# ctu-vras/monoforce

Hardware: AMD Instinct MI355X
Metric: rollout-steps/sec (batch x horizon) on 256x256 terrain (higher is better)
Workload: dtype f32; 1 GPU; c3: B=1024/GPU x T=500 x N=4 contact points, 256x256 grid (res 0.05 m), one shared terrain+friction map (the same on every rank), integrator=odeint-euler (reference default), forward+backward; BASE...; rollouts_per_gpu=1024, rollouts_total=1024, horizon=500, contact_points=4, parallelism=rollout-sharded x1

## Files before the change

monoforce_amd/csrc/rollout_fwd_cp_kernel.h:

```cpp
#pragma once
#include "rollout_cp_common.h"
#include "rollout_fwd_kernel.h"
#include <type_traits>

namespace mf {

template <typename S, int INTEG, bool FORCES, bool ZMU, bool REC, bool LOSS = false>
__global__ void __launch_bounds__(256) __attribute__((amdgpu_waves_per_eu(1, 2))) rollout_fwd_cp_kernel(const RolloutArgs<S> a) {
  using namespace cp;
  using M = Mth<S, std::is_same<S, float>::value>;
  using Msk = typename MaskOf<S>::type;
  constexpr unsigned kS = (unsigned)sizeof(S);
  const int tid = blockIdx.x * blockDim.x + threadIdx.x;
  const int b = (tid >> 4) + a.b0;
  if (b >= a.B) return;
  if (a.loss_poison != nullptr && tid == 0) a.loss_poison[0] = (S)__builtin_nanf("");
  const int p = (tid >> 2) & 3;
  const int q = tid & 3;
  const int cc = q < 3 ? q : 2;
  const S one = S(1.0), zero = S(0.0);
  const int HW = a.H * a.W, last = HW - 1;
  const bool has_mu = a.mu != nullptr;
  const unsigned moff = a.map_shared ? 0u : (unsigned)b * (unsigned)HW;
  const S* zmap = a.z;
  const S* mumap = has_mu ? a.mu : a.z;

  const bool act = p < a.N;
  const int pi = act ? p : 0;
  const S P0 = a.points[pi * 3 + 0], P1 = a.points[pi * 3 + 1], P2 = a.points[pi * 3 + 2];
  const int part = act ? a.part[pi] : -1;
  const S tv_v = part < 0 ? zero : one;
  const S tv_w = part < 0 ? zero : ((part & 1) ? a.half_ly : -a.half_ly);
  const S I0 = a.Iinv[cc * 3 + 0], I1 = a.Iinv[cc * 3 + 1], I2 = a.Iinv[cc * 3 + 2];
  const S grav_c = cc == 2 ? a.mg * a.inv_mass : zero;
  const int cell_off = ((q & 1) ? a.H : 0) + ((q & 2) ? 1 : 0);
  const S wa_s = (q & 2) ? one : -one, wa_o = (q & 2) ? zero : one;
  const S wb_s = (q & 1) ? one : -one, wb_o = (q & 1) ? zero : one;
  const S n_mul = q < 2 ? -a.inv_res : zero, n_add = q < 2 ? zero : one;

  S x, xd, w, R0, R1, R2;
  if (a.default_state) {
    const S v0 = a.controls[(size_t)b * a.ctrl_sb + 0], w0 = a.controls[(size_t)b * a.ctrl_sb + 1];
    x = zero; xd = cc == 0 ? v0 : zero; w = cc == 2 ? w0 : zero;
    R0 = cc == 0 ? one : zero; R1 = cc == 1 ? one : zero; R2 = cc == 2 ? one : zero;
    if (p == 0) {
      S* oxd = const_cast<S*>(a.xd0); S* oR = const_cast<S*>(a.R0); S* ow = const_cast<S*>(a.w0);
      a.x0[b * 3 + cc] = x; oxd[b * 3 + cc] = xd; ow[b * 3 + cc] = w;
      oR[b * 9 + cc * 3 + 0] = R0; oR[b * 9 + cc * 3 + 1] = R1; oR[b * 9 + cc * 3 + 2] = R2;
    }
  } else {
    x = a.x0[b * 3 + cc]; xd = a.xd0[b * 3 + cc]; w = a.w0[b * 3 + cc];
    R0 = a.R0[b * 9 + cc * 3 + 0]; R1 = a.R0[b * 9 + cc * 3 + 1]; R2 = a.R0[b * 9 + cc * 3 + 2];
  }

  auto footprint = [&](S pc, int* idx, S* wq, S* ou = nullptr) {
    const S lim = S(262144.0);
    const S u = M::cell_coord(pc, a.d_max, a.res, a.inv_res);
    const int ui = (int)M::clamp(u, -lim, lim);
    const S fr = u - (S)ui;
    const int base = dppi<kB1>(ui) + __mul24(a.H, dppi<kB0>(ui));
    *idx = min(max(base + cell_off, 0), last);
    const S wa = mf_fma(wa_s, dpp<kB0>(fr), wa_o), wb = mf_fma(wb_s, dpp<kB1>(fr), wb_o);
    *wq = wa * wb;
    if (ou) *ou = u;
  };

  if (!a.skip_snap) {
    const S pc = (P0 * R0 + P1 * R1 + P2 * R2) + x;
    int idx; S wq;
    footprint(pc, &idx, &wq);
    const S zq = dot4(wq, ld32(zmap, moff + (unsigned)idx));
    const S acc = sum_points(act ? zq : zero);
    const S xz = acc / (S)a.N;
    x = cc == 2 ? xz : x;
    if (p == 0 && q == 2) a.x0[b * 3 + 2] = xz;
  }

  const unsigned row_stride = (a.layout == MF_LAYOUT_TIME_MAJOR) ? (unsigned)a.B : 1u;
  const unsigned row0 = (a.layout == MF_LAYOUT_TIME_MAJOR) ? (unsigned)b : (unsigned)b * (unsigned)a.T;
  S* v3base = p == 0 ? a.Xs : p == 1 ? a.Xds : p == 2 ? a.Om : (a.Xraw ? a.Xraw : a.Xs);
  const S sink_l = (p == 3 && a.Xraw) ? zero : a.sink;
  const Msk m_xd = p == 1 ? ~(Msk)0 : (Msk)0, m_w = p == 2 ? ~(Msk)0 : (Msk)0;
  char* p3 = reinterpret_cast<char*>(v3base) + (size_t)(row0 * 3u + (unsigned)cc) * kS;
  const Rsrc rCtrl = make_rsrc(a.controls);
  unsigned o9 = (row0 * 9u + (unsigned)cc * 3u) * kS;
  const unsigned frow = (unsigned)a.fstride * 3u;
  unsigned ofs = (row0 * frow + (unsigned)p * 3u + (unsigned)cc) * kS, off = ofs;
  const unsigned d3 = row_stride * 3u * kS, d9 = row_stride * 9u * kS, df = row_stride * frow * kS;
  const char* pRs = reinterpret_cast<const char*>(a.Rs);
  const char* pFs = reinterpret_cast<const char*>(a.Fs);
  const char* pFf = reinterpret_cast<const char*>(a.Ff);

  S oFs = zero, oFf = zero;

  auto emit_row = [&](S ex, S exd, S ew, S e0, S e1, S e2, unsigned adv) {
    const S vx = mf_fma(e2, sink_l, ex);
    const S v3 = bfi(m_w, ew, bfi(m_xd, exd, vx));
    __builtin_nontemporal_store(v3, reinterpret_cast<S*>(p3));
    bstore3(pRs, o9, 0u, e0, e1, e2);
    if (FORCES) { bstore1(pFs, ofs, 0u, oFs); bstore1(pFf, off, 0u, oFf); }
    if (adv) { p3 += d3; o9 += d9; ofs += df; off += df; }
  };

  const int n_steps = (INTEG == MF_INTEG_ODEINT_EULER) ? a.T - 1 : a.T;
  unsigned v_ctrl = (unsigned)b * (unsigned)a.ctrl_sb * kS;
  S cv, cw;
  bload2(rCtrl, v_ctrl, 0u, &cv, &cw);
  S h_ode = (INTEG == MF_INTEG_ODEINT_EULER && a.T > 1) ? a.ts[1] - a.ts[0] : zero;
  struct Geo { S r, pc, wq, zc, mc, e, u, il, coln2; int idx; };
  auto geometry = [&](S gx, S g0, S g1, S g2) {
    Geo g;
    g.r = cp_body_r(P0, P1, P2, g0, g1, g2);
    g.pc = g.r + gx;
    footprint(g.pc, &g.idx, &g.wq, &g.u);
    const int idx = g.idx;
    if constexpr (ZMU) {
      const Pk2<S> zm = *reinterpret_cast<const Pk2<S>*>(reinterpret_cast<const char*>(a.zmu) + (size_t)((unsigned)idx * 2u * kS));
      g.zc = zm.a; g.mc = zm.b;
    } else {
      g.zc = ld32(zmap, moff + (unsigned)idx);
      g.mc = ld32(mumap, moff + (unsigned)idx);
    }
    g.coln2 = dot3(g0, g0);
    g.il = M::inv_len(g.coln2);
    g.e = g0 * g.il;
    return g;
  };
  char* const pRec0 = reinterpret_cast<char*>(a.rec);
  unsigned rec_off = (unsigned)tid * kRecBytesPerLane<S>;
  const unsigned rec_step = (unsigned)a.B * 16u * kRecBytesPerLane<S>;
  typedef S f4v __attribute__((ext_vector_type(4)));
  auto rec_store = [&](const f4v& rq, unsigned adv) {
#if defined(MF_REC_NOSTORE)
    asm volatile("" :: "v"(rq));
#elif defined(MF_REC_PLAIN)
    *reinterpret_cast<f4v*>(pRec0 + (size_t)rec_off) = rq;
#else
    __builtin_nontemporal_store(rq, reinterpret_cast<f4v*>(pRec0 + (size_t)rec_off));
#endif
    if (adv) rec_off += rec_step;
  };
  auto contact = [&](const Geo& g, S vxd, S vw, S tv, S* xdd, S* wd, S* oFr, S* oFf, f4v* rq) {
    const S vp = cp_vel(vxd, vw, g.r);
    const S zq = dot4(g.wq, g.zc);
    const S mub = dot4(g.wq, has_mu ? g.mc : one);
    const S dz = g.zc - dpp<kB0>(g.zc);
    const S u = mf_fma(dpp<kN12>(dz), n_mul, n_add);
    const S inl = M::inv_len(dot3(u, u));
    const S nrm = u * inl;
    const S dh = dpp<kB2>(g.pc) - zq;
    S cj = M::sigmoid_m10(dh);
    cj = act ? cj : zero;
    const S csum = sum_points(cj);
    const S inv_csum = M::div(one, csum);
    const S vn = dot3(vp, nrm);
    const S A = cp_normal_force(a.k, dh, a.damp, vn);
    const S Fr = M::clamp(cp_spring(A, nrm, cj, inv_csum), -a.mg, a.mg);
    const S Nn = M::sqrt(dot3(Fr, Fr));
    const S s = mub * cp_cmd(tv, g.e, vp);
    const S sn = dot3(s, nrm);
    const S Ff = M::clamp(Nn * cp_tangent(s, sn, nrm), -a.mg, a.mg);
    const S f = Fr + Ff;
    const S tau = unrot(cross_pre(g.r, f));
    const S Fsum = sum_points(f), Tsum = sum_points(tau);
    const S wraw = cp_wraw(I0, I1, I2, Tsum);
    *wd = M::clamp(wraw, -a.omega_max, a.omega_max);
    *xdd = Fsum * a.inv_mass - grav_c;
    *oFr = Fr; *oFf = Ff;
    if constexpr (REC) *rq = f4v{g.u, cj, wraw, A};
  };

  S l_acc = zero;
  int l_j = 0;
  const int l_last = LOSS ? a.loss_T2 - 1 : 0;
  const unsigned l_lane = LOSS ? ((unsigned)b * (unsigned)a.loss_T2 * 3u + (unsigned)cc) : 0u;
  struct Stamp { S g, w; };
  auto loss_peek = [&](int row) {
    Stamp st = {zero, zero};
    if constexpr (LOSS) {
      st.g = ld32(a.loss_gt, l_lane + (unsigned)(min(l_j, l_last) * 3));
      st.w = a.loss_row_w[row];
    }
    return st;
  };
  auto loss_row = [&](S ex, S e2, const Stamp& st) {
    if constexpr (LOSS) {
      const S term = cp_loss_term(mf_fma(e2, a.sink, ex), st.g, st.w);
      l_acc += st.w != zero ? term : zero;
      l_j += st.w != zero ? 1 : 0;
    }
  };

  if constexpr (INTEG == MF_INTEG_ODEINT_EULER) {
    S t_cur = a.T > 1 ? a.ts[1] : zero;
    const unsigned ctrl_step = (unsigned)a.ctrl_st * kS, v_ctrl_last = v_ctrl + (unsigned)(a.T - 1) * ctrl_step;
    unsigned v_ts = kS;
    asm("" : "+v"(v_ts));
    const unsigned v_ts_last = (unsigned)max(a.T - 1, 0) * kS;
    auto ode_step = [&](int n, const Geo& g, Geo& g_next, S cv_n, S cw_n, S h, S& cv_next, S& cw_next, S& h_next) {
      v_ctrl = min(v_ctrl + ctrl_step, v_ctrl_last);
      bload2(rCtrl, v_ctrl, 0u, &cv_next, &cw_next);
      v_ts = min(v_ts + kS, v_ts_last);
      const S t_next = *reinterpret_cast<const S*>(reinterpret_cast<const char*>(a.ts) + (size_t)v_ts);
      const Stamp stamp = loss_peek(n + 1);
      const S tv = cp_track(tv_v, tv_w, cv_n, cw_n);
      const S d0 = h * cross_pre(w, R0), d1 = h * cross_pre(w, R1), d2 = h * cross_pre(w, R2);
      const S xn = mf_fma(h, xd, x);
      const S Rn0 = R0 + unrot(d0), Rn1 = R1 + unrot(d1), Rn2 = R2 + unrot(d2);
      g_next = geometry(xn, Rn0, Rn1, Rn2);
      emit_row(x, xd, w, R0, R1, R2, 1u);
      x = xn; R0 = Rn0; R1 = Rn1; R2 = Rn2;
      S xdd, wd, Fr, Ff;
      f4v rq;
      contact(g, xd, w, tv, &xdd, &wd, &Fr, &Ff, &rq);
      if constexpr (REC) rec_store(rq, 1u);
      xd = mf_fma(h, xdd, xd);
      w = mf_fma(h, wd, w);
      oFs = mf_fma(h, Fr, oFs);
      oFf = mf_fma(h, Ff, oFf);
      h_next = t_next - t_cur;
      t_cur = t_next;
      loss_row(x, R2, stamp);
    };
    Geo gA, gB;
    S cvA = cv, cwA = cw, hA = h_ode, cvB = zero, cwB = zero, hB = zero;
    if (n_steps > 0) gA = geometry(x, R0, R1, R2);
    loss_row(x, R2, loss_peek(0));
    __builtin_amdgcn_s_waitcnt(0);
    int n = 0;
    for (; n + 1 < n_steps; n += 2) {
      ode_step(n, gA, gB, cvA, cwA, hA, cvB, cwB, hB);
      ode_step(n + 1, gB, gA, cvB, cwB, hB, cvA, cwA, hA);
    }
    if (n < n_steps) ode_step(n, gA, gB, cvA, cwA, hA, cvB, cwB, hB);
  } else {
    __builtin_amdgcn_s_waitcnt(0);
    for (int n = 0; n < n_steps; ++n) {
      const int nn = min(n + 1, a.T - 1);
      S cv_next, cw_next;
      bload2(rCtrl, v_ctrl, __builtin_amdgcn_readfirstlane((unsigned)(nn * a.ctrl_st) * kS), &cv_next, &cw_next);
      const S tv = cp_track(tv_v, tv_w, cv, cw);
      S xdd, wd, Fr, Ff;
      const Geo g = geometry(x, R0, R1, R2);
      emit_row(x, xd, w, R0, R1, R2, n > 0 ? 1u : 0u);
      f4v rq;
      contact(g, xd, w, tv, &xdd, &wd, &Fr, &Ff, &rq);
      if constexpr (REC) rec_store(rq, 1u);
      const S h = a.dt;
      xd = mf_fma(xdd, h, xd);
      x = mf_fma(xd, h, x);
      w = mf_fma(wd, h, w);
      const S th2 = dot3(w, w);
      const S il = M::inv_len(th2);
      const S kc = w * il;
      const S k1 = dpp<kRot1>(kc), k2 = dpp<kRot2>(kc);
      S sn_, oc;
      M::sincos_small(M::len_of(th2, il) * h, &sn_, &oc);
      const S kk = M::kReciprocalNorm ? th2 * (il * il) : dot3(kc, kc);
      const S ock = oc * kc;
      const S m0 = one + oc * (kc * kc - kk);
      const S m1 = mf_fma(ock, k1, -(sn_ * k2));
      const S m2 = mf_fma(ock, k2, sn_ * k1);
      const S n0 = R0 * dpp<kB0>(m0) + R1 * dpp<kB1>(m2) + R2 * dpp<kB2>(m1);
      const S n1 = R0 * dpp<kB0>(m1) + R1 * dpp<kB1>(m0) + R2 * dpp<kB2>(m2);
      const S n2 = R0 * dpp<kB0>(m2) + R1 * dpp<kB1>(m1) + R2 * dpp<kB2>(m0);
      R0 = n0; R1 = n1; R2 = n2;
      oFs = Fr; oFf = Ff;
      cv = cv_next; cw = cw_next;
    }
  }
  if (n_steps > 0 || INTEG == MF_INTEG_ODEINT_EULER) emit_row(x, xd, w, R0, R1, R2, 1u);
  if constexpr (LOSS) {
    static_assert(!LOSS || INTEG == MF_INTEG_ODEINT_EULER, "the fused loss rides on the default integrator's kernels");
    __shared__ S l_sh[80];
    const int lane = threadIdx.x;
    if (lane < 16) l_sh[lane] = zero;
    if (p == 0 && q < 3) l_sh[(lane >> 4) * 4 + q] = l_acc;
    __syncthreads();
    unsigned last = 0u;
    if (lane == 0) {
      S tot = zero;
#pragma unroll
      for (int r = 0; r < 4; ++r) tot += (l_sh[r * 4 + 0] + l_sh[r * 4 + 1]) + l_sh[r * 4 + 2];
      __builtin_nontemporal_store(tot, a.loss_partial + blockIdx.x);
      __threadfence();
      last = atomicAdd(a.loss_ticket, 1u) == gridDim.x - 1 ? 1u : 0u;
    }
    last = __builtin_amdgcn_readfirstlane(last);
    if (last) {
      __threadfence();
      const int n_act = min(64, (a.B - (int)blockIdx.x * 4) * 16);
      S tot = zero;
      for (unsigned k2 = (unsigned)lane; k2 < gridDim.x; k2 += (unsigned)n_act) tot += __builtin_nontemporal_load(a.loss_partial + k2);
      l_sh[16 + lane] = tot;
      __syncthreads();
      if (lane == 0) {
        S sum = zero;
        for (int k2 = 0; k2 < n_act; ++k2) sum += l_sh[16 + k2];
        a.loss_out[0] = sum * a.loss_inv_count;
        *a.loss_ticket = 0u;
      }
    }
  }
}

int launch_rollout_fwd_cp_f32(const RolloutArgs<float>& a, const FwdRoute& r, int integ, hipStream_t st);
int launch_rollout_fwd_cp_f64(const RolloutArgs<double>& a, const FwdRoute& r, int integ, hipStream_t st);
template <typename S>
int launch_rollout_fwd_cp_t(const RolloutArgs<S>& a, const FwdRoute& r, int integ, hipStream_t st) {
  const int block = r.block;
  const unsigned grid = (unsigned)(((long long)a.B * 16 + block - 1) / block);
  const bool forces = r.forces, zmu = r.zmu;
  const bool rec = r.record;
  if (r.loss == kLossInLaunch) {
    constexpr int I = MF_INTEG_ODEINT_EULER;
    if (rec) { if (zmu) MF_KLAUNCH((rollout_fwd_cp_kernel<S, I, false, true, true, true>), dim3(grid), dim3(block), 0, st, a);
               else MF_KLAUNCH((rollout_fwd_cp_kernel<S, I, false, false, true, true>), dim3(grid), dim3(block), 0, st, a); }
    else     { if (zmu) MF_KLAUNCH((rollout_fwd_cp_kernel<S, I, false, true, false, true>), dim3(grid), dim3(block), 0, st, a);
               else MF_KLAUNCH((rollout_fwd_cp_kernel<S, I, false, false, false, true>), dim3(grid), dim3(block), 0, st, a); }
    hipError_t e = hipGetLastError();
    MF_REQUIRE(e == hipSuccess, MF_ERR_LAUNCH, std::string("rollout_fwd (component-parallel, fused loss) launch: ") + hipGetErrorString(e));
    return MF_OK;
  }
#define MF_CP(INTEG_, FORCES_, ZMU_) do { if (rec) MF_KLAUNCH((rollout_fwd_cp_kernel<S, INTEG_, FORCES_, ZMU_, true>), dim3(grid), dim3(block), 0, st, a); \
                                          else MF_KLAUNCH((rollout_fwd_cp_kernel<S, INTEG_, FORCES_, ZMU_, false>), dim3(grid), dim3(block), 0, st, a); } while (0)
#define MF_CP_F(INTEG_)                                          \
  do {                                                           \
    if (forces) { if (zmu) MF_CP(INTEG_, true, true); else MF_CP(INTEG_, true, false); }    \
    else        { if (zmu) MF_CP(INTEG_, false, true); else MF_CP(INTEG_, false, false); }  \
  } while (0)
  if (integ == MF_INTEG_DYNAMICS) MF_CP_F(MF_INTEG_DYNAMICS); else MF_CP_F(MF_INTEG_ODEINT_EULER);
#undef MF_CP_F
#undef MF_CP
  hipError_t e = hipGetLastError();
  MF_REQUIRE(e == hipSuccess, MF_ERR_LAUNCH, std::string("rollout_fwd (component-parallel) launch: ") + hipGetErrorString(e));
  return MF_OK;
}


}
```

monoforce_amd/csrc/rollout_fwd_kernel.h:

```cpp
#pragma once
#include <cstdlib>
#include "rollout_common.h"
#include "rollout_route.h"

namespace mf {

template <typename S>
struct RolloutArgs {
  int B, T, N, H, W, n_tracks, layout, map_shared, skip_snap, fstride, default_state, ctrl_sb, ctrl_st, b0;
  S mass, inv_mass, mg, k, damp, omega_max, res, inv_res, d_max, dt, half_ly, sink;
  S Iinv[9];
  const S* z;
  const S* mu;
  const S* controls;
  const S* ts;
  const S* points;
  const int* part;
  S* x0;
  const S* xd0;
  const S* R0;
  const S* w0;
  S* Xs;
  S* Xds;
  S* Rs;
  S* Om;
  S* Fs;
  S* Ff;
  S* Xraw;
  const S* joint_angles;
  S joint_xyz[12];
  S* cost_rows;
  int pose_stride;
  S* path_cost;
  const S* zmu;
  S* rec;
  int loss_T2;
  const S* loss_gt;
  const S* loss_row_w;
  S* loss_partial;
  unsigned* loss_ticket;
  S* loss_out;
  S loss_inv_count;
  S* loss_poison;
};

template <typename S, bool FAST>
struct Mth {
  static __device__ __forceinline__ S div(S a, S b) { return a / b; }
  static __device__ __forceinline__ S cell_coord(S q, S d_max, S res, S) { return (q + d_max) / res; }
  static __device__ __forceinline__ S sqrt(S v) { return mf_sqrt(v); }
  static __device__ __forceinline__ S sigmoid_m10(S dh) { return (S)1 / ((S)1 + mf_exp((S)10 * dh)); }
  static __device__ __forceinline__ S inv_len(S len2) { return (S)1 / mf_max(mf_sqrt(len2), (S)1e-6); }
  static __device__ __forceinline__ S len_of(S len2, S) { return mf_sqrt(len2); }
  static constexpr bool kReciprocalNorm = false;
  static __device__ __forceinline__ void sincos_small(S v, S* s, S* omc) { S c; mf_sincos(v, s, &c); *omc = (S)1 - c; }
  static __device__ __forceinline__ S clamp(S v, S lo, S hi) { return mf_clamp(v, lo, hi); }
  static __device__ __forceinline__ void sincos(S v, S* sn, S* cs) { mf_sincos(v, sn, cs); }
};
template <>
struct Mth<float, true> {
  static __device__ __forceinline__ float div(float a, float b) { return a * __builtin_amdgcn_rcpf(b); }
  static __device__ __forceinline__ float cell_coord(float q, float d_max, float res, float inv_res) {
    const float a = q + d_max;
    const float u = a * inv_res;
    return fmaf(fmaf(-u, res, a), inv_res, u);
  }
  static __device__ __forceinline__ float sqrt(float v) { return __builtin_amdgcn_sqrtf(v); }
  static __device__ __forceinline__ float sigmoid_m10(float dh) {
    return __builtin_amdgcn_rcpf(1.0f + __builtin_amdgcn_exp2f(14.426950408889634f * dh));
  }
  static __device__ __forceinline__ float inv_len(float len2) { return __builtin_amdgcn_rsqf(fmaxf(len2, 1e-12f)); }
  static __device__ __forceinline__ float len_of(float len2, float il) { return len2 * il; }
  static constexpr bool kReciprocalNorm = true;
  static __device__ __forceinline__ float clamp(float v, float lo, float hi) { return __builtin_amdgcn_fmed3f(v, lo, hi); }
  static __device__ __forceinline__ void sincos(float v, float* sn, float* cs) { *sn = __sinf(v); *cs = __cosf(v); }
  static __device__ __forceinline__ void sincos_small(float v, float* s, float* omc) {
    const float v2 = v * v;
    const float ts = v * (1.0f + v2 * (-1.0f / 6 + v2 * (1.0f / 120 - v2 * (1.0f / 5040))));
    const float tc = v2 * (0.5f + v2 * (-1.0f / 24 + v2 * (1.0f / 720 - v2 * (1.0f / 40320))));
    const float rev = __builtin_amdgcn_fractf(v * 0.15915494309189535f);
    const bool small = fabsf(v) < 0.25f;
    *s = small ? ts : __builtin_amdgcn_sinf(rev);
    *omc = small ? tc : 1.0f - __builtin_amdgcn_cosf(rev);
  }
};

template <typename S, bool FAST>
__device__ __forceinline__ Cell<S> locate_m(S qx, S qy, S d_max, S res, S inv_res, int H, int last) {
  const S lim = (S)262144.0;
  S ux = Mth<S, FAST>::cell_coord(qx, d_max, res, inv_res);
  S uy = Mth<S, FAST>::cell_coord(qy, d_max, res, inv_res);
  int ix = (int)Mth<S, FAST>::clamp(ux, -lim, lim);
  int iy = (int)Mth<S, FAST>::clamp(uy, -lim, lim);
  Cell<S> c;
  c.fx = ux - (S)ix;
  c.fy = uy - (S)iy;
  int base = iy + __mul24(H, ix);
  c.ic = min(max(base, 0), last);
  c.i_f = min(max(base + H, 0), last);
  c.il = min(max(base + 1, 0), last);
  c.ifl = min(max(base + 1 + H, 0), last);
  return c;
}

template <typename S>
__device__ __forceinline__ S ld32(const S* base, unsigned elem) {
  return *reinterpret_cast<const S*>(reinterpret_cast<const char*>(base) + (size_t)(elem * (unsigned)sizeof(S)));
}

template <typename S>
struct CellPair { S a, b; };
template <typename S>
__device__ __forceinline__ void gather4(const S* map, unsigned moff, const Cell<S>& c, int last, S (&v)[4]) {
  const int p1 = min(c.ic, last - 1), p2 = min(c.i_f, last - 1);
  const CellPair<S> q1 = *reinterpret_cast<const CellPair<S>*>(reinterpret_cast<const char*>(map) + (size_t)((moff + (unsigned)p1) * (unsigned)sizeof(S)));
  const CellPair<S> q2 = *reinterpret_cast<const CellPair<S>*>(reinterpret_cast<const char*>(map) + (size_t)((moff + (unsigned)p2) * (unsigned)sizeof(S)));
  v[0] = c.ic != p1 ? q1.b : q1.a;
  v[2] = c.il != p1 ? q1.b : q1.a;
  v[1] = c.i_f != p2 ? q2.b : q2.a;
  v[3] = c.ifl != p2 ? q2.b : q2.a;
}

template <typename S>
struct CellQuad { S za, ma, zb, mb; };
template <typename S>
__device__ __forceinline__ void gather4x2(const S* zmu, const Cell<S>& c, int last, S (&z)[4], S (&m)[4]) {
  const int p1 = min(c.ic, last - 1), p2 = min(c.i_f, last - 1);
  const CellQuad<S> q1 = *reinterpret_cast<const CellQuad<S>*>(reinterpret_cast<const char*>(zmu) + (size_t)((unsigned)p1 * (unsigned)(2 * sizeof(S))));
  const CellQuad<S> q2 = *reinterpret_cast<const CellQuad<S>*>(reinterpret_cast<const char*>(zmu) + (size_t)((unsigned)p2 * (unsigned)(2 * sizeof(S))));
  const bool ec = c.ic != p1, el = c.il != p1, ef = c.i_f != p2, efl = c.ifl != p2;
  z[0] = ec ? q1.zb : q1.za;   m[0] = ec ? q1.mb : q1.ma;
  z[2] = el ? q1.zb : q1.za;   m[2] = el ? q1.mb : q1.ma;
  z[1] = ef ? q2.zb : q2.za;   m[1] = ef ? q2.mb : q2.ma;
  z[3] = efl ? q2.zb : q2.za;  m[3] = efl ? q2.mb : q2.ma;
}

template <typename S, int G, int PPL, bool FAST = false>
__device__ __forceinline__ void articulate_body(GroupSum<G, S>& gs, const S* ja, const S* joint_xyz, S mp, const S (&P0)[PPL][3],
                                                const int (&part)[PPL], const bool (&act)[PPL], S (&P)[PPL][3], S (&Iv)[9]) {
  const S one = (S)1, zero = (S)0;
  S sj[4], cj4[4];
#pragma unroll
  for (int q = 0; q < 4; ++q) Mth<S, FAST>::sincos(ja[q], &sj[q], &cj4[q]);
  S I6[6] = {zero, zero, zero, zero, zero, zero};
#pragma unroll
  for (int j = 0; j < PPL; ++j) {
    const int q = max(part[j], 0);
    const S sn = sj[q], cs = cj4[q];
    const S jx = joint_xyz[q * 3 + 0], jz = joint_xyz[q * 3 + 2];
    const S dx = P0[j][0] - jx, dz = P0[j][2] - jz;
    const S rx = (dx * cs + dz * sn) + jx, rz = (-(dx * sn) + dz * cs) + jz;
    P[j][0] = part[j] >= 0 ? rx : P0[j][0];
    P[j][1] = P0[j][1];
    P[j][2] = part[j] >= 0 ? rz : P0[j][2];
    const S px = P[j][0], py = P[j][1], pzz = P[j][2];
    const S wgt = act[j] ? mp : zero;
    I6[0] += wgt * (py * py + pzz * pzz); I6[1] += wgt * (px * px + pzz * pzz); I6[2] += wgt * (px * px + py * py);
    I6[3] -= wgt * px * py; I6[4] -= wgt * px * pzz; I6[5] -= wgt * py * pzz;
  }
  gs.sum_n(I6);
  const S a00 = I6[0], a11 = I6[1], a22 = I6[2], a01 = I6[3], a02 = I6[4], a12 = I6[5];
  const S c00 = a11 * a22 - a12 * a12, c01 = a02 * a12 - a01 * a22, c02 = a01 * a12 - a02 * a11;
  const S c11 = a00 * a22 - a02 * a02, c12 = a01 * a02 - a00 * a12, c22 = a00 * a11 - a01 * a01;
  const S idet = Mth<S, FAST>::div(one, a00 * c00 + a01 * c01 + a02 * c02);
  Iv[0] = c00 * idet; Iv[1] = c01 * idet; Iv[2] = c02 * idet;
  Iv[3] = c01 * idet; Iv[4] = c11 * idet; Iv[5] = c12 * idet;
  Iv[6] = c02 * idet; Iv[7] = c12 * idet; Iv[8] = c22 * idet;
}

template <typename S, int G, int PPL, int INTEG, bool FAST, bool JOINTS = false, bool FORCES = true, int COST = 0, bool SPLIT = false, bool ZMU = false, bool REC = false>
__global__ void __launch_bounds__(G > 256 ? G : 256) rollout_fwd_kernel(const RolloutArgs<S> a) {
  using M = Mth<S, FAST>;
  const int tid = blockIdx.x * blockDim.x + threadIdx.x;
  const int b = tid / G + a.b0;
  const int gl = tid % G;
  if (b >= a.B) return;
  const S one = (S)1, zero = (S)0;
  const int HW = a.H * a.W, last = HW - 1;
  const bool has_mu = a.mu != nullptr;
  __shared__ S gs_lds[G > 64 ? 2 * (G / 64) * kGroupSumMaxValues : 1];
  GroupSum<G, S> gs;
  gs.lds = gs_lds;
  const unsigned moff = a.map_shared ? 0u : (unsigned)b * (unsigned)HW;
  const S* zmap = a.z;
  const S* mumap = has_mu ? a.mu : a.z;

  S P[PPL][3];
  S P0[PPL][3];
  S Iv[9];
  int part[PPL];
  bool act[PPL];
#pragma unroll
  for (int j = 0; j < PPL; ++j) {
    int i = gl * PPL + j;
    act[j] = i < a.N;
    int ii = act[j] ? i : 0;
    P[j][0] = a.points[ii * 3 + 0];
    P[j][1] = a.points[ii * 3 + 1];
    P[j][2] = a.points[ii * 3 + 2];
    part[j] = act[j] ? a.part[ii] : -1;
#pragma unroll
    for (int c = 0; c < 3; ++c) P0[j][c] = P[j][c];
  }
#pragma unroll
  for (int c = 0; c < 9; ++c) Iv[c] = a.Iinv[c];

  S x[3], xd[3], R[9], w[3];
  if (a.default_state) {
    const S v0 = a.controls[(size_t)b * a.ctrl_sb + 0], w0 = a.controls[(size_t)b * a.ctrl_sb + 1];
#pragma unroll
    for (int c = 0; c < 3; ++c) { x[c] = zero; xd[c] = c == 0 ? v0 : zero; w[c] = c == 2 ? w0 : zero; }
#pragma unroll
    for (int c = 0; c < 9; ++c) R[c] = (c % 4 == 0) ? one : zero;
    if (gl == 0) {
      S* oxd = const_cast<S*>(a.xd0); S* oR = const_cast<S*>(a.R0); S* ow = const_cast<S*>(a.w0);
#pragma unroll
      for (int c = 0; c < 3; ++c) { a.x0[b * 3 + c] = x[c]; oxd[b * 3 + c] = xd[c]; ow[b * 3 + c] = w[c]; }
#pragma unroll
      for (int c = 0; c < 9; ++c) oR[b * 9 + c] = R[c];
    }
  } else {
#pragma unroll
    for (int c = 0; c < 3; ++c) {
      x[c] = a.x0[b * 3 + c];
      xd[c] = a.xd0[b * 3 + c];
      w[c] = a.w0[b * 3 + c];
    }
#pragma unroll
    for (int c = 0; c < 9; ++c) R[c] = a.R0[b * 9 + c];
  }

  if (!a.skip_snap) {
    S acc = zero;
#pragma unroll
    for (int j = 0; j < PPL; ++j) {
      S px = P[j][0] * R[0] + P[j][1] * R[1] + P[j][2] * R[2] + x[0];
      S py = P[j][0] * R[3] + P[j][1] * R[4] + P[j][2] * R[5] + x[1];
      Cell<S> c = locate_m<S, FAST>(px, py, a.d_max, a.res, a.inv_res, a.H, last);
      S z4[4];
      gather4(zmap, moff, c, last, z4);
      S v = blend(c, z4[0], z4[1], z4[2], z4[3]);
      acc += act[j] ? v : zero;
    }
    acc = gs.sum(acc);
    x[2] = acc / (S)a.N;
    if (gl == 0) a.x0[b * 3 + 2] = x[2];
  }

  const size_t row_stride = (a.layout == MF_LAYOUT_TIME_MAJOR) ? (size_t)a.B : 1;
  const size_t row0 = (a.layout == MF_LAYOUT_TIME_MAJOR) ? (size_t)b : (size_t)b * a.T;
  S* pXs = a.Xs + row0 * 3;
  S* pXds = a.Xds + row0 * 3;
  S* pOm = a.Om + row0 * 3;
  S* pRs = a.Rs + row0 * 9;
  S* pXraw = (a.Xraw ? a.Xraw : a.Xs) + row0 * 3;
  const size_t frow = (size_t)a.fstride * 3;
  S* pFs = a.Fs + row0 * frow + (size_t)gl * PPL * 3;
  S* pFf = a.Ff + row0 * frow + (size_t)gl * PPL * 3;

  S oFs[PPL][3], oFf[PPL][3];
#pragma unroll
  for (int j = 0; j < PPL; ++j)
#pragma unroll
    for (int c = 0; c < 3; ++c) oFs[j][c] = oFf[j][c] = zero;

  S* pC = COST ? a.cost_rows + row0 * 4 : nullptr;
  const int role = gl & 3;
  const bool role_b0 = (role & 1) != 0, role_b1 = (role & 2) != 0;
  const S sink_l = (role == 0 && a.Xraw) ? zero : a.sink;
  S* pV3 = role == 0 ? pXraw : role == 1 ? pXs : role == 2 ? pXds : pOm;
  S* pRrow = pRs + 3 * min(role, 2);
  int pose_wait = 0;
  S pc_n = zero, pc_mean = zero, pc_m2 = zero;
  auto store_pose = [&]() {
    pXs[0] = x[0] + R[2] * a.sink; pXs[1] = x[1] + R[5] * a.sink; pXs[2] = x[2] + R[8] * a.sink;
#pragma unroll
    for (int c = 0; c < 9; ++c) pRs[c] = R[c];
  };
  const S inv_N = one / (S)a.N, inv_Nm1 = one / (S)max(a.N - 1, 1);
  auto emit_row = [&](size_t adv) {
#ifdef MF_DBG_NOSTORE
    if (a.B > 0) return;
#endif
    if (COST) {
      auto stc = [](S* p, S v) { __builtin_nontemporal_store(v, p); };
      S nrm_j[PPL], nsum = zero;
#pragma unroll
      for (int j = 0; j < PPL; ++j) {
        nrm_j[j] = M::sqrt(oFs[j][0] * oFs[j][0] + oFs[j][1] * oFs[j][1] + oFs[j][2] * oFs[j][2]);
        nsum += act[j] ? nrm_j[j] : zero;
      }
      const S mean = gs.sum(nsum) * inv_N;
      S dsum = zero;
#pragma unroll
      for (int j = 0; j < PPL; ++j) { const S dv = nrm_j[j] - mean; dsum += act[j] ? dv * dv : zero; }
      const S sdev = M::sqrt(gs.sum(dsum) * inv_Nm1);
      S r20 = R[6], r21 = R[7], r22 = R[8];
      if (INTEG == MF_INTEG_ODEINT_EULER && COST == 2) {
        const S half = (S)0.5;
        const S c00 = R[4] * R[8] - R[5] * R[7], c01 = R[5] * R[6] - R[3] * R[8], c02 = R[3] * R[7] - R[4] * R[6];
        const S c10 = R[2] * R[7] - R[1] * R[8], c11 = R[0] * R[8] - R[2] * R[6], c12 = R[1] * R[6] - R[0] * R[7];
        const S c20 = R[1] * R[5] - R[2] * R[4], c21 = R[2] * R[3] - R[0] * R[5], c22 = R[0] * R[4] - R[1] * R[3];
        const S hid = M::div(half, R[0] * c00 + R[1] * c01 + R[2] * c02);
        const S Y[9] = {half * R[0] + hid * c00, half * R[1] + hid * c01, half * R[2] + hid * c02,
                        half * R[3] + hid * c10, half * R[4] + hid * c11, half * R[5] + hid * c12,
                        half * R[6] + hid * c20, half * R[7] + hid * c21, half * R[8] + hid * c22};
        const S d20 = Y[1] * Y[5] - Y[2] * Y[4], d21 = Y[2] * Y[3] - Y[0] * Y[5], d22 = Y[0] * Y[4] - Y[1] * Y[3];
        const S hid2 = M::div(half, Y[6] * d20 + Y[7] * d21 + Y[8] * d22);
        r20 = half * Y[6] + hid2 * d20; r21 = half * Y[7] + hid2 * d21; r22 = half * Y[8] + hid2 * d22;
      }
      stc(pC + 0, r20); stc(pC + 1, r21); stc(pC + 2, r22); stc(pC + 3, sdev);
      pC += adv * 4;
      const S wgt = adv ? one : zero;
      pc_n += wgt;
      const S dlt = sdev - pc_mean;
      pc_mean += wgt * M::div(dlt, mf_max(pc_n, one));
      pc_m2 += wgt * dlt * (sdev - pc_mean);
      return;
    }
    auto st = [](S* p, S v) { __builtin_nontemporal_store(v, p); };
    if (SPLIT && G >= 4) {
      S v3[3], rr[3];
#pragma unroll
      for (int c = 0; c < 3; ++c) {
        const S t0 = x[c] + R[3 * c + 2] * sink_l;
        const S t1 = role_b0 ? w[c] : xd[c];
        v3[c] = role_b1 ? t1 : t0;
        const S r0 = role_b0 ? R[3 + c] : R[c];
        rr[c] = role_b1 ? R[6 + c] : r0;
      }
      st(pV3 + 0, v3[0]); st(pV3 + 1, v3[1]); st(pV3 + 2, v3[2]);
      st(pRrow + 0, rr[0]); st(pRrow + 1, rr[1]); st(pRrow + 2, rr[2]);
      pV3 += adv * 3; pRrow += adv * 9;
      if (FORCES) {
#pragma unroll
        for (int j = 0; j < PPL; ++j)
#pragma unroll
          for (int c = 0; c < 3; ++c) st(pFs + j * 3 + c, oFs[j][c]);
#pragma unroll
        for (int j = 0; j < PPL; ++j)
#pragma unroll
          for (int c = 0; c < 3; ++c) st(pFf + j * 3 + c, oFf[j][c]);
        pFs += adv * frow; pFf += adv * frow;
      }
      return;
    }
#ifdef MF_NO_SHARED_STATE_STORES
    constexpr bool kShare = false;
#else
    constexpr bool kShare = FAST && G > 64 && PPL == 1 && !JOINTS;
#endif
    const int wv = kShare ? __builtin_amdgcn_readfirstlane((int)(threadIdx.x >> 6)) : 0;
    constexpr int kNW = G > 64 ? G / 64 : 1;
    const bool do_x = !kShare || wv == 0, do_v = !kShare || wv == (kNW > 2 ? 1 : 0), do_R = !kShare || wv == (kNW > 2 ? 2 : 1);
    if (do_x) {
      st(pXraw + 0, x[0]); st(pXraw + 1, x[1]); st(pXraw + 2, x[2]);
      st(pXs + 0, x[0] + R[2] * a.sink);
      st(pXs + 1, x[1] + R[5] * a.sink);
      st(pXs + 2, x[2] + R[8] * a.sink);
    }
    if (do_v) {
      st(pXds + 0, xd[0]); st(pXds + 1, xd[1]); st(pXds + 2, xd[2]);
      st(pOm + 0, w[0]); st(pOm + 1, w[1]); st(pOm + 2, w[2]);
    }
    if (do_R) {
#pragma unroll
      for (int c = 0; c < 9; ++c) st(pRs + c, R[c]);
    }
    pXs += adv * 3; pXds += adv * 3; pOm += adv * 3; pRs += adv * 9; pXraw += adv * 3;
    if (FORCES) {
#pragma unroll
      for (int j = 0; j < PPL; ++j)
// ... 604 lines not shown
```

Before: 1.463 billion rollout-steps/s.

## Micro-optimize contact step: DPP torque, med3 clamp, mu specialization, unclamped control loads

Bundles several instruction-level tweaks in the rollout forward kernel. The torque unrotation is folded into a DPP-fused inverse-inertia product written in inline asm, and the index clamp uses a single med3. The inactive-point mask is folded into the sigmoid denominator by using infinity, and the has_mu branch is hoisted into a compile-time tag. The Euler loop is restructured to load timestamps as a packed triple and to drop per-step clamping of the control and timestamp offsets by using offset buffer resources. These changes aim to shorten the per-step dependency chain and cut VALU and SALU work, at the cost of more inline asm and more code duplication.

```diff
diff --git a/monoforce_amd/csrc/rollout_fwd_cp_kernel.h b/monoforce_amd/csrc/rollout_fwd_cp_kernel.h
--- a/monoforce_amd/csrc/rollout_fwd_cp_kernel.h
+++ b/monoforce_amd/csrc/rollout_fwd_cp_kernel.h
@@ -4,6 +4,24 @@
 #include <type_traits>
 
 namespace mf {
+
+namespace cp {
+__device__ __forceinline__ float cp_wraw_rot(float I0, float I1, float I2, float Trot) {
+  float acc = I0 * dpp<kB1>(Trot);
+  asm("v_fmac_f32_dpp %0, %1, %2 quad_perm:[2,2,2,2] row_mask:0xf bank_mask:0xf bound_ctrl:1\n\t"
+      "v_fmac_f32_dpp %0, %1, %3 quad_perm:[0,0,0,0] row_mask:0xf bank_mask:0xf bound_ctrl:1"
+      : "+v"(acc) : "v"(Trot), "v"(I1), "v"(I2));
+  return acc;
+}
+__device__ __forceinline__ double cp_wraw_rot(double I0, double I1, double I2, double Trot) {
+  return mf_fma(I2, dpp<kB0>(Trot), mf_fma(I1, dpp<kB2>(Trot), I0 * dpp<kB1>(Trot)));
+}
+__device__ __forceinline__ int clamp_index(int v, int last) {
+  int r;
+  asm("v_med3_i32 %0, %1, 0, %2" : "=v"(r) : "v"(v), "v"(last));
+  return r;
+}
+}
 
 template <typename S, int INTEG, bool FORCES, bool ZMU, bool REC, bool LOSS = false>
 __global__ void __launch_bounds__(256) __attribute__((amdgpu_waves_per_eu(1, 2))) rollout_fwd_cp_kernel(const RolloutArgs<S> a) {
@@ -20,6 +38,8 @@
   const int cc = q < 3 ? q : 2;
   const S one = S(1.0), zero = S(0.0);
   const int HW = a.H * a.W, last = HW - 1;
+  int Hv = a.H;
+  asm("" : "+v"(Hv));
   const bool has_mu = a.mu != nullptr;
   const unsigned moff = a.map_shared ? 0u : (unsigned)b * (unsigned)HW;
   const S* zmap = a.z;
@@ -27,6 +47,7 @@
 
   const bool act = p < a.N;
   const int pi = act ? p : 0;
+  const S den1 = act ? one : (S)__builtin_inff();
   const S P0 = a.points[pi * 3 + 0], P1 = a.points[pi * 3 + 1], P2 = a.points[pi * 3 + 2];
   const int part = act ? a.part[pi] : -1;
   const S tv_v = part < 0 ? zero : one;
@@ -58,8 +79,8 @@
     const S u = M::cell_coord(pc, a.d_max, a.res, a.inv_res);
     const int ui = (int)M::clamp(u, -lim, lim);
     const S fr = u - (S)ui;
-    const int base = dppi<kB1>(ui) + __mul24(a.H, dppi<kB0>(ui));
-    *idx = min(max(base + cell_off, 0), last);
+    const int base = dppi<kB1>(ui) + __mul24(dppi<kB0>(ui), Hv);
+    *idx = clamp_index(base + cell_off, last);
     const S wa = mf_fma(wa_s, dpp<kB0>(fr), wa_o), wb = mf_fma(wb_s, dpp<kB1>(fr), wb_o);
     *wq = wa * wb;
     if (ou) *ou = u;
@@ -118,8 +139,8 @@
       const Pk2<S> zm = *reinterpret_cast<const Pk2<S>*>(reinterpret_cast<const char*>(a.zmu) + (size_t)((unsigned)idx * 2u * kS));
       g.zc = zm.a; g.mc = zm.b;
     } else {
+      g.mc = ld32(mumap, moff + (unsigned)idx);
       g.zc = ld32(zmap, moff + (unsigned)idx);
-      g.mc = ld32(mumap, moff + (unsigned)idx);
     }
     g.coln2 = dot3(g0, g0);
     g.il = M::inv_len(g.coln2);
@@ -140,17 +161,16 @@
 #endif
     if (adv) rec_off += rec_step;
   };
-  auto contact = [&](const Geo& g, S vxd, S vw, S tv, S* xdd, S* wd, S* oFr, S* oFf, f4v* rq) {
+  auto contact = [&](auto mu_tag, const Geo& g, S vxd, S vw, S tv, S* xdd, S* wd, S* oFr, S* oFf, f4v* rq) {
     const S vp = cp_vel(vxd, vw, g.r);
     const S zq = dot4(g.wq, g.zc);
-    const S mub = dot4(g.wq, has_mu ? g.mc : one);
+    const S mub = dot4(g.wq, decltype(mu_tag)::value ? g.mc : one);
     const S dz = g.zc - dpp<kB0>(g.zc);
     const S u = mf_fma(dpp<kN12>(dz), n_mul, n_add);
     const S inl = M::inv_len(dot3(u, u));
     const S nrm = u * inl;
     const S dh = dpp<kB2>(g.pc) - zq;
-    S cj = M::sigmoid_m10(dh);
-    cj = act ? cj : zero;
+    const S cj = M::sigmoid_m10(dh, den1);
     const S csum = sum_points(cj);
     const S inv_csum = M::div(one, csum);
     const S vn = dot3(vp, nrm);
@@ -161,9 +181,9 @@
     const S sn = dot3(s, nrm);
     const S Ff = M::clamp(Nn * cp_tangent(s, sn, nrm), -a.mg, a.mg);
     const S f = Fr + Ff;
-    const S tau = unrot(cross_pre(g.r, f));
+    const S tau = cross_pre(g.r, f);
     const S Fsum = sum_points(f), Tsum = sum_points(tau);
-    const S wraw = cp_wraw(I0, I1, I2, Tsum);
+    const S wraw = cp_wraw_rot(I0, I1, I2, Tsum);
     *wd = M::clamp(wraw, -a.omega_max, a.omega_max);
     *xdd = Fsum * a.inv_mass - grav_c;
     *oFr = Fr; *oFf = Ff;
@@ -193,15 +213,24 @@
 
   if constexpr (INTEG == MF_INTEG_ODEINT_EULER) {
     S t_cur = a.T > 1 ? a.ts[1] : zero;
-    const unsigned ctrl_step = (unsigned)a.ctrl_st * kS, v_ctrl_last = v_ctrl + (unsigned)(a.T - 1) * ctrl_step;
+    const unsigned ctrl_step = (unsigned)a.ctrl_st * kS;
     unsigned v_ts = kS;
     asm("" : "+v"(v_ts));
     const unsigned v_ts_last = (unsigned)max(a.T - 1, 0) * kS;
-    auto ode_step = [&](int n, const Geo& g, Geo& g_next, S cv_n, S cw_n, S h, S& cv_next, S& cw_next, S& h_next) {
-      v_ctrl = min(v_ctrl + ctrl_step, v_ctrl_last);
+    const char* const pTs = reinterpret_cast<const char*>(a.ts);
+    const Rsrc rCtrl1 = rCtrl + ctrl_step, rCtrl2 = rCtrl1 + ctrl_step;
+    auto next_ctrl = [&](S& cv_next, S& cw_next) {
+      v_ctrl += ctrl_step;
       bload2(rCtrl, v_ctrl, 0u, &cv_next, &cw_next);
+    };
+    auto next_stamp_clamped = [&]() {
       v_ts = min(v_ts + kS, v_ts_last);
-      const S t_next = *reinterpret_cast<const S*>(reinterpret_cast<const char*>(a.ts) + (size_t)v_ts);
+      const S t_next = *reinterpret_cast<const S*>(pTs + (size_t)v_ts);
+      const S h_new = t_next - t_cur;
+      t_cur = t_next;
+      return h_new;
+    };
+    auto ode_step = [&](auto mu_tag, int n, const Geo& g, Geo& g_next, S cv_n, S cw_n, S h, S h_new, S& h_next) __attribute__((always_inline)) {
       const Stamp stamp = loss_peek(n + 1);
       const S tv = cp_track(tv_v, tv_w, cv_n, cw_n);
       const S d0 = h * cross_pre(w, R0), d1 = h * cross_pre(w, R1), d2 = h * cross_pre(w, R2);
@@ -212,14 +241,13 @@
       x = xn; R0 = Rn0; R1 = Rn1; R2 = Rn2;
       S xdd, wd, Fr, Ff;
       f4v rq;
-      contact(g, xd, w, tv, &xdd, &wd, &Fr, &Ff, &rq);
+      contact(mu_tag, g, xd, w, tv, &xdd, &wd, &Fr, &Ff, &rq);
       if constexpr (REC) rec_store(rq, 1u);
       xd = mf_fma(h, xdd, xd);
       w = mf_fma(h, wd, w);
       oFs = mf_fma(h, Fr, oFs);
       oFf = mf_fma(h, Ff, oFf);
-      h_next = t_next - t_cur;
-      t_cur = t_next;
+      h_next = h_new;
       loss_row(x, R2, stamp);
     };
     Geo gA, gB;
@@ -227,15 +255,34 @@
     if (n_steps > 0) gA = geometry(x, R0, R1, R2);
     loss_row(x, R2, loss_peek(0));
     __builtin_amdgcn_s_waitcnt(0);
-    int n = 0;
-    for (; n + 1 < n_steps; n += 2) {
-      ode_step(n, gA, gB, cvA, cwA, hA, cvB, cwB, hB);
-      ode_step(n + 1, gB, gA, cvB, cwB, hB, cvA, cwA, hA);
-    }
-    if (n < n_steps) ode_step(n, gA, gB, cvA, cwA, hA, cvB, cwB, hB);
+    const int n_pairs = a.T >= 4 ? (a.T - 2) >> 1 : 0;
+    auto run = [&](auto mu_tag) __attribute__((always_inline)) {
+      for (int n = 0; n < 2 * n_pairs; n += 2) {
+        const Pk3<S> tt = *reinterpret_cast<const Pk3<S>*>(pTs + (size_t)v_ts);
+        bload2(rCtrl1, v_ctrl, 0u, &cvB, &cwB);
+        ode_step(mu_tag, n, gA, gB, cvA, cwA, hA, tt.b - tt.a, hB);
+        bload2(rCtrl2, v_ctrl, 0u, &cvA, &cwA);
+        v_ctrl += 2u * ctrl_step;
+        v_ts += 2u * kS;
+        t_cur = tt.c;
+        ode_step(mu_tag, n + 1, gB, gA, cvB, cwB, hB, tt.c - tt.b, hA);
+      }
+      const int n = 2 * n_pairs;
+      if (n < n_steps) {
+        const S h_a = next_stamp_clamped();
+        next_ctrl(cvB, cwB);
+        ode_step(mu_tag, n, gA, gB, cvA, cwA, hA, h_a, hB);
+        if (n + 1 < n_steps) {
+          const S h_b = next_stamp_clamped();
+          next_ctrl(cvA, cwA);
+          ode_step(mu_tag, n + 1, gB, gA, cvB, cwB, hB, h_b, hA);
+        }
+      }
+    };
+    if (has_mu) run(std::true_type{}); else run(std::false_type{});
   } else {
     __builtin_amdgcn_s_waitcnt(0);
-    for (int n = 0; n < n_steps; ++n) {
+    auto dyn_step = [&](auto mu_tag, int n) __attribute__((always_inline)) {
       const int nn = min(n + 1, a.T - 1);
       S cv_next, cw_next;
       bload2(rCtrl, v_ctrl, __builtin_amdgcn_readfirstlane((unsigned)(nn * a.ctrl_st) * kS), &cv_next, &cw_next);
@@ -244,7 +291,7 @@
       const Geo g = geometry(x, R0, R1, R2);
       emit_row(x, xd, w, R0, R1, R2, n > 0 ? 1u : 0u);
       f4v rq;
-      contact(g, xd, w, tv, &xdd, &wd, &Fr, &Ff, &rq);
+      contact(mu_tag, g, xd, w, tv, &xdd, &wd, &Fr, &Ff, &rq);
       if constexpr (REC) rec_store(rq, 1u);
       const S h = a.dt;
       xd = mf_fma(xdd, h, xd);
@@ -267,7 +314,9 @@
       R0 = n0; R1 = n1; R2 = n2;
       oFs = Fr; oFf = Ff;
       cv = cv_next; cw = cw_next;
-    }
+    };
+    if (has_mu) { for (int n = 0; n < n_steps; ++n) dyn_step(std::true_type{}, n); }
+    else { for (int n = 0; n < n_steps; ++n) dyn_step(std::false_type{}, n); }
   }
   if (n_steps > 0 || INTEG == MF_INTEG_ODEINT_EULER) emit_row(x, xd, w, R0, R1, R2, 1u);
   if constexpr (LOSS) {
diff --git a/monoforce_amd/csrc/rollout_fwd_kernel.h b/monoforce_amd/csrc/rollout_fwd_kernel.h
--- a/monoforce_amd/csrc/rollout_fwd_kernel.h
+++ b/monoforce_amd/csrc/rollout_fwd_kernel.h
@@ -50,6 +50,7 @@
   static __device__ __forceinline__ S cell_coord(S q, S d_max, S res, S) { return (q + d_max) / res; }
   static __device__ __forceinline__ S sqrt(S v) { return mf_sqrt(v); }
   static __device__ __forceinline__ S sigmoid_m10(S dh) { return (S)1 / ((S)1 + mf_exp((S)10 * dh)); }
+  static __device__ __forceinline__ S sigmoid_m10(S dh, S den1) { return (S)1 / (den1 + mf_exp((S)10 * dh)); }
   static __device__ __forceinline__ S inv_len(S len2) { return (S)1 / mf_max(mf_sqrt(len2), (S)1e-6); }
   static __device__ __forceinline__ S len_of(S len2, S) { return mf_sqrt(len2); }
   static constexpr bool kReciprocalNorm = false;
@@ -68,6 +69,9 @@
   static __device__ __forceinline__ float sqrt(float v) { return __builtin_amdgcn_sqrtf(v); }
   static __device__ __forceinline__ float sigmoid_m10(float dh) {
     return __builtin_amdgcn_rcpf(1.0f + __builtin_amdgcn_exp2f(14.426950408889634f * dh));
+  }
+  static __device__ __forceinline__ float sigmoid_m10(float dh, float den1) {
+    return __builtin_amdgcn_rcpf(den1 + __builtin_amdgcn_exp2f(14.426950408889634f * dh));
   }
   static __device__ __forceinline__ float inv_len(float len2) { return __builtin_amdgcn_rsqf(fmaxf(len2, 1e-12f)); }
   static __device__ __forceinline__ float len_of(float len2, float il) { return len2 * il; }
```

New measurement: 1.508 billion rollout-steps/s, median of 6. +3.0%, better.
